# junliu111/CV-MonoSLAM

Measured on AMD Instinct MI355X. Metric: srukf_updates_per_sec, higher is better.
Workload: dtype f64; 1 GPU; BASELINE configs[2]: 200 inverse-depth landmarks (n=1204, Na=1209, L=2419), M=N matched, fp64, one batched refactor per frame, synthetic 640x480 figure-8 sequence; landmarks=200, state_dim=1204, sequences_per_gpu=1, update_mode=batched

## Files before the change

cv-monoslam_amd/csrc/srukf_rank.hip:

```cpp
#include <hip/hip_runtime.h>
#include "srukf_device.h"
#include "srukf_rank.h"
#include "srukf_motion.h"
#include "srukf_motion_reduce.h"
#include "srukf_launch.h"

__global__ __launch_bounds__(256) void k_rank_shadow(int n, int ld, int r, const double* __restrict__ S, const int* __restrict__ perm, double* __restrict__ A)
{
    const int a = blockIdx.x;
    double* out = A + (size_t)a * ld;
    if (a >= r) { for (int b = threadIdx.x; b < ld; b += 256) out[b] = 0.0; return; }
    const double* src = S + (size_t)perm[a] * ld;
    for (int b = threadIdx.x; b < ld; b += 256) out[b] = (b >= a && b < n) ? src[perm[b]] : 0.0;
}

__global__ __launch_bounds__(256) void k_row_energy(int n, int ld, const double* __restrict__ S, double* __restrict__ e)
{
    __shared__ double red[16];
    const int k = blockIdx.x;
    double v[1] = { 0.0 };
    for (int i = k + threadIdx.x; i < n; i += 256) { const double s = S[(size_t)k * ld + i]; v[0] += s * s; }
    block_sum<1>(v, red);
    if (threadIdx.x == 0) e[k] = v[0];
}

__global__ __launch_bounds__(256) void k_rank_diag(int n, int ld, const double* __restrict__ G, const int* __restrict__ perm, double* __restrict__ gdiag)
{
    const int a = blockIdx.x * 256 + threadIdx.x;
    if (a < n) { const int j = perm[a]; gdiag[a] = G[(size_t)j * ld + j]; }
}

template <int MODE>
__device__ __forceinline__ void rank_expand_body(int n, int ld, int r, double eps, const double* __restrict__ Sp, const double* __restrict__ D,
                                                 const int* __restrict__ perm, const int* __restrict__ iperm, const double* __restrict__ gdiag,
                                                 FrameScalars* __restrict__ fs, const double* __restrict__ X, int do_traj, double* __restrict__ S,
                                                 double* __restrict__ A, double* __restrict__ sigR, double gamma,
                                                 const KDims& d, const KWeights& w,
                                                 const srukf_params& p, double* __restrict__ Z, double* __restrict__ DZ, int f32, const int bid, const StepExport& ex, const double null_rel = 0.0,
                                                 unsigned int* __restrict__ fold_sync = nullptr, const int fold_words = 0)
{
    constexpr bool PROJ = MODE == 2;
    auto rnd = [&](double v) { return f32 ? (double)(float)v : v; };
    extern __shared__ double lrow[];
    __shared__ double prow[2][8];
    __shared__ double red[16 * 3];
    const int j = bid;
    const int Na = n + 5;
    const bool table = sigR && fs->ctl_next_valid && !fs->frozen;
    auto table_rows = [&](const int i, const int sg, const double (&srow)[4], const double (&mnoise)[3], const bool isnull) {
        const MotionCtl mc = { fs->ctl[0], fs->ctl[1], fs->ctl[2], fs->ctl[3], fs->ctl[4] };
        const double xr[4] = { X[n - 4], X[n - 3], X[n - 2], X[n - 1] };
        double rr[4], c2, s2;
        if (isnull) srukf_motion_centre(mc, xr, rr, c2, s2);
        else srukf_motion_point(mc, xr, srow, mnoise, sg ? -gamma : gamma, rr, c2, s2);
        double4* o = reinterpret_cast<double4*>(sigR + (size_t)(1 + sg * Na + i) * 8);
        o[0] = make_double4(rr[0], rr[1], rr[2], rr[3]); o[1] = make_double4(c2, s2, 0.0, 0.0);
        if constexpr (PROJ) { double* q = prow[sg]; q[0] = rr[0]; q[1] = rr[1]; q[2] = rr[2]; q[3] = rr[3]; q[4] = c2; q[5] = s2; }
    };
    const double f1 = PROJ ? p.cam_f / p.cam_dx : 0.0, f2 = PROJ ? p.cam_f / p.cam_dy : 0.0;
    auto project_pair = [&](const int i, const int k, const double (&dev)[6], const double e0, const double e1, const double* r0, const double* r1, const int dzrow) {
        double base[6];
#pragma unroll
        for (int e = 0; e < 6; e++) base[e] = X[6 * k + e];
        double zp[2], zm[2];
        srukf_project_sigma(p, f1, f2, base, dev, e0, e1, gamma, r0, zp[0], zp[1]);
        srukf_project_sigma(p, f1, f2, base, dev, e0, e1, -gamma, r1, zm[0], zm[1]);
        *reinterpret_cast<double2*>(Z + (size_t)(1 + i) * d.mp + 2 * k) = make_double2(zp[0], zp[1]);
        *reinterpret_cast<double2*>(Z + (size_t)(1 + Na + i) * d.mp + 2 * k) = make_double2(zm[0], zm[1]);
        if (dzrow >= 0) *reinterpret_cast<double2*>(DZ + (size_t)dzrow * d.mp + 2 * k) = make_double2(zp[0] - zm[0], zp[1] - zm[1]);
    };
    if constexpr (PROJ) {
        const int nchk = (n - r + SRUKF_RANK_COLS - 1) / SRUKF_RANK_COLS;
        if (j > n + nchk) {
            if (!table) return;
            const int q = j - n - nchk - 1;
            if (threadIdx.x < 2) {
                const double zero4[4] = { 0, 0, 0, 0 };
                double mnoise[3] = { 0, 0, 0 };
                if (q < 3) mnoise[q] = fs->ctl[5 + q];
                table_rows(n + q, threadIdx.x, zero4, mnoise, false);
            }
            __syncthreads();
            const double zero6[6] = { 0, 0, 0, 0, 0, 0 };
            const double e0 = (q == 3) ? p.sigma_measure : 0.0, e1 = (q == 4) ? p.sigma_measure : 0.0;
            for (int k = threadIdx.x; k < d.N; k += 256) project_pair(n + q, k, zero6, e0, e1, prow[0], prow[1], -1);
            return;
        }
    }
    if (j == n) {
        if (fold_sync) {
            const int base = (fold_words + FOLD_FLAG_STRIDE - 1) / FOLD_FLAG_STRIDE * FOLD_FLAG_STRIDE;
            for (int q = threadIdx.x; q < fold_words; q += 256) fold_sync[q] = 0u;
            if (threadIdx.x < 2 + SRUKF_STAT_GROUPS) fold_sync[base + FOLD_FLAG_STRIDE * threadIdx.x] = 0u;
        }
        if (table && threadIdx.x < (PROJ ? 1 : 11)) {
            const double zero4[4] = { 0, 0, 0, 0 };
            if (threadIdx.x == 0) {
                const MotionCtl mc = { fs->ctl[0], fs->ctl[1], fs->ctl[2], fs->ctl[3], fs->ctl[4] };
                const double xr[4] = { X[n - 4], X[n - 3], X[n - 2], X[n - 1] };
                double s0[4], c0s, s0s;
                srukf_motion_centre(mc, xr, s0, c0s, s0s);
                double4* o = reinterpret_cast<double4*>(sigR);
                o[0] = make_double4(s0[0], s0[1], s0[2], s0[3]); o[1] = make_double4(c0s, s0s, 0.0, 0.0);
                if constexpr (PROJ) { double* q = prow[0]; q[0] = s0[0]; q[1] = s0[1]; q[2] = s0[2]; q[3] = s0[3]; q[4] = c0s; q[5] = s0s; }
            } else {
                const int q = (threadIdx.x - 1) >> 1, sg = (threadIdx.x - 1) & 1;
                double mnoise[3] = { 0, 0, 0 };
                if (q < 3) mnoise[q] = fs->ctl[5 + q];
                table_rows(n + q, sg, zero4, mnoise, false);
            }
        }
        if constexpr (PROJ) {
            __syncthreads();
            if (table) {
                const double f1c = p.cam_f / p.cam_dx, f2c = p.cam_f / p.cam_dy;
                for (int k = threadIdx.x; k < d.N; k += 256) {
                    double base[6];
#pragma unroll
                    for (int e = 0; e < 6; e++) base[e] = X[6 * k + e];
                    double ox, oy;
                    srukf_project(p, f1c, f2c, base, prow[0][0], prow[0][1], prow[0][2], prow[0][4], prow[0][5], 0.0, 0.0, ox, oy);
                    *reinterpret_cast<double2*>(Z + 2 * k) = make_double2(ox, oy);
                }
            }
        }
        const int bx = iperm[n - 4], by = iperm[n - 3];
        double v[3] = { 0, 0, 0 };
        for (int a = threadIdx.x; a < r; a += 256) {
            const double p = (bx >= a) ? rnd(Sp[(size_t)a * ld + bx]) : 0.0, q = (by >= a) ? rnd(Sp[(size_t)a * ld + by]) : 0.0;
            v[0] += p * p; v[1] += p * q; v[2] += q * q;
        }
        block_sum<3>(v, red);
        if (ex.dst) {
            __shared__ double red4[16 * 10];
            int bc[4];
#pragma unroll
            for (int e = 0; e < 4; e++) bc[e] = iperm[n - 4 + e];
            double v4[10];
#pragma unroll
            for (int q = 0; q < 10; q++) v4[q] = 0.0;
            for (int a = threadIdx.x; a < r; a += 256) {
                double s4[4];
#pragma unroll
                for (int e = 0; e < 4; e++) s4[e] = (bc[e] >= a) ? rnd(Sp[(size_t)a * ld + bc[e]]) : 0.0;
                int q = 0;
#pragma unroll
                for (int e = 0; e < 4; e++)
#pragma unroll
                    for (int g = e; g < 4; g++) v4[q++] += s4[e] * s4[g];
            }
            block_sum<10>(v4, red4);
            if (threadIdx.x == 0) {
                int q = 0;
                for (int e = 0; e < 4; e++)
                    for (int g = e; g < 4; g++) { st_dev(ex.view + 4 * e + g, v4[q]); st_dev(ex.view + 4 * g + e, v4[q]); q++; }
                for (int e = 0; e < 4; e++) st_dev(ex.view + 16 + e, X[n - 4 + e]);
            }
        }
        if (threadIdx.x == 0 && do_traj) {
            double* traj = fs->traj_base;
            if (traj) {
                double* t = traj + (size_t)8 * fs->frame;
                for (int e = 0; e < 4; e++) t[e] = X[n - 4 + e];
                t[4] = v[0]; t[5] = v[1]; t[6] = v[1]; t[7] = v[2];
            }
            if (ex.dst) {
                __hip_atomic_store(&fs->frame, fs->frame + 1, __ATOMIC_RELAXED, __HIP_MEMORY_SCOPE_AGENT);
                __hip_atomic_store(&fs->const_rows_pending, 1, __ATOMIC_RELAXED, __HIP_MEMORY_SCOPE_AGENT);
            } else {
                fs->frame += 1;
                fs->const_rows_pending = 1;
            }
            if (!sigR) srukf_prepare_control(fs);
        }
        return;
    }
    if (j > n) {
        const int a = r + SRUKF_RANK_COLS * (j - n - 1) + (threadIdx.x & 15), kl = threadIdx.x >> 4;
        __shared__ double cs[16][17];
        cs[kl][threadIdx.x & 15] = (a < n) ? srukf_rank_colsq(Sp, ld, r, a, kl) : 0.0;
        __syncthreads();
        if (threadIdx.x < 16 && a < n) {
            double t = 0.0;
            for (int q = 0; q < 16; q++) t += cs[q][threadIdx.x];
            if (gdiag[a] - t > 1e-12 + null_rel * fabs(gdiag[a])) { atomicAdd(&fs->clamp_rows, 1); atomicMin(&fs->clamp_first, perm[a]); }
        }
        return;
    }
    const int a = j;
    const int jj = perm[a];
    double* out = S + (size_t)jj * ld;
    if (table && threadIdx.x < 2) {
        double srow[4] = { 0, 0, 0, 0 };
        const double zero3[3] = { 0, 0, 0 };
        if (a < r) {
#pragma unroll
            for (int e = 0; e < 4; e++) srow[e] = (r - 4 + e >= a) ? rnd(Sp[(size_t)a * ld + (r - 4 + e)]) : 0.0;
        }
        table_rows(jj, threadIdx.x, srow, zero3, a >= r);
    }
    if (a >= r) {
        if constexpr (PROJ) {
            if (table) {
                __syncthreads();
                if (threadIdx.x < 2) {
                    const int k = jj / 6, sg = threadIdx.x;
                    double dev[6], base[6];
#pragma unroll
                    for (int e = 0; e < 6; e++) { dev[e] = (6 * k + e == jj) ? rnd(sqrt(eps)) : 0.0; base[e] = X[6 * k + e]; }
                    double ox, oy;
                    srukf_project_sigma(p, f1, f2, base, dev, 0.0, 0.0, sg ? -gamma : gamma, prow[sg], ox, oy);
                    *reinterpret_cast<double2*>(Z + (size_t)(1 + sg * Na + jj) * d.mp + 2 * k) = make_double2(ox, oy);
                    const double pox = __shfl_xor(ox, 1), poy = __shfl_xor(oy, 1);
                    if (sg == 0) *reinterpret_cast<double2*>(DZ + (size_t)a * d.mp + 2 * k) = make_double2(ox - pox, oy - poy);
                }
            }
        }
        if (sigR && fs->const_rows_ok) return;
        for (int c = threadIdx.x; c < ld; c += 256) out[c] = (c == jj) ? rnd(sqrt(eps)) : 0.0;
        return;
    }
    const double* src = Sp + (size_t)a * ld;
    double* sh = A ? A + (size_t)a * ld : nullptr;
    double mx = 0.0;
    for (int b0 = (sigR ? (a & ~3) : 0) + threadIdx.x; b0 < ld; b0 += 4 * 256) {
        double sv[4]; int cc[4];
#pragma unroll
        for (int u = 0; u < 4; u++) {
            const int b = b0 + 256 * u;
            sv[u] = (b >= a && b < n) ? src[b] : 0.0;
            cc[u] = (b < n) ? perm[b] : b;
        }
#pragma unroll
        for (int u = 0; u < 4; u++) {
            const int b = b0 + 256 * u;
            if (b >= ld) break;
            const bool upper = b >= a && b < n && cc[u] >= jj;
            if (upper && cc[u] > jj) mx = fmax(mx, fabs(sv[u]));
            const double rv = rnd(sv[u]);
            if (sh) sh[b] = rv;
            if constexpr (PROJ) lrow[b] = rv;
            if (upper || !sigR) out[cc[u]] = upper ? rv : 0.0;
        }
    }
    mx = wave_max(mx);
    if ((threadIdx.x & 63) == 0) red[threadIdx.x >> 6] = mx;
    __syncthreads();
    if (threadIdx.x == 0) {
        mx = fmax(fmax(red[0], red[1]), fmax(red[2], red[3]));
        const double gamma = __longlong_as_double((long long)fs->gmax_bits);
        const double xi = __longlong_as_double((long long)fs->ximax_bits);
        const double nu = fmax(1.0, sqrt((double)n * n - 1.0));
        const double beta2 = fmax(fmax(gamma, xi / nu), 1e-15);
        const double dj = D[a];
        const double th = mx * sqrt(dj);
        if (th * th / beta2 > dj) { atomicAdd(&fs->clamp_rows, 1); atomicMin(&fs->clamp_first, jj); }
    }
    if constexpr (PROJ) {
        if (table) {
            for (int k = threadIdx.x; k < d.N; k += 256) {
                double dev[6];
#pragma unroll
                for (int e = 0; e < 6; e++) { const int col = 6 * k + e; dev[e] = (col >= jj) ? lrow[iperm[col]] : 0.0; }
                project_pair(jj, k, dev, 0.0, 0.0, prow[0], prow[1], a);
            }
        }
    }
}

template <int MODE>
__global__ __launch_bounds__(256) void k_rank_expand(int n, int ld, int r, double eps, const double* __restrict__ Sp, const double* __restrict__ D,
                                                     const int* __restrict__ perm, const int* __restrict__ iperm, const double* __restrict__ gdiag,
                                                     FrameScalars* __restrict__ fs, const double* __restrict__ X, int do_traj, double* __restrict__ S,
                                                     double* __restrict__ A, double* __restrict__ sigR, double gamma,
                                                     KDims d, KWeights w,
                                                     srukf_params p, double* __restrict__ Z, double* __restrict__ DZ, int f32, StepExport ex, double null_rel,
                                                     unsigned int* __restrict__ fold_sync, int fold_words)
{
    const int extra = (int)gridDim.x - n;
    const int bid = (int)blockIdx.x < extra ? n + (int)blockIdx.x : (int)blockIdx.x - extra;
    rank_expand_body<MODE>(n, ld, r, eps, Sp, D, perm, iperm, gdiag, fs, X, do_traj, S, A, sigR, gamma, d, w, p, Z, DZ, f32, bid, ex, null_rel, fold_sync, fold_words);
    if (!ex.dst) return;
    const int ncount = extra + r;
    if ((int)blockIdx.x >= ncount) return;
    __shared__ int last;
    asm volatile("s_waitcnt vmcnt(0)" ::: "memory");
    __syncthreads();
    if (threadIdx.x == 0) {
        const int g = (int)blockIdx.x & 63, gsize = (ncount - g + 63) >> 6, groups = ncount < 64 ? ncount : 64;
        int* c1 = ex.cnt + 64 * g;
        last = 0;
        if (__hip_atomic_fetch_add(c1, 1, __ATOMIC_RELAXED, __HIP_MEMORY_SCOPE_AGENT) == gsize - 1) {
            __hip_atomic_store(c1, 0, __ATOMIC_RELAXED, __HIP_MEMORY_SCOPE_AGENT);
            if (__hip_atomic_fetch_add(&fs->export_cnt, 1, __ATOMIC_RELAXED, __HIP_MEMORY_SCOPE_AGENT) == groups - 1) {
                __hip_atomic_store(&fs->export_cnt, 0, __ATOMIC_RELAXED, __HIP_MEMORY_SCOPE_AGENT);
                last = 1;
            }
        }
    }
    __syncthreads();
    if (!last) return;
    const unsigned long long* fw = (const unsigned long long*)fs;
    for (int i = threadIdx.x; i < ex.nfs; i += 256) ex.dst[i] = __hip_atomic_load(fw + i, __ATOMIC_RELAXED, __HIP_MEMORY_SCOPE_AGENT);
    if (threadIdx.x < 20) ((double*)(ex.dst + ex.nfs))[threadIdx.x] = ld_dev(ex.view + threadIdx.x);
    __threadfence_system();
    __syncthreads();
    if (threadIdx.x == 0) {
        if (ex.set && __hip_atomic_load(&fs->clamp_rows, __ATOMIC_RELAXED, __HIP_MEMORY_SCOPE_AGENT) == 0) {
            for (int e = 0; e < 6; e++) ex.odo[e] = ex.poses[e];
            srukf_step_scalars(fs, ex.odo, 1, ex.a, false);
        }
        if (ex.flag) __hip_atomic_store(ex.flag, ex.seq, __ATOMIC_RELEASE, __HIP_MEMORY_SCOPE_SYSTEM);
    }
}
__global__ __launch_bounds__(256) void k_rank_expand_b(int n, int ld, int r, double eps, const ExpandArgs* __restrict__ tab, int per, double gamma, KDims d, KWeights w, srukf_params p)
{
    const int f = (int)blockIdx.x / per, bid = (int)blockIdx.x - f * per;
    const ExpandArgs a = tab[f];
    rank_expand_body<2>(n, ld, r, eps, a.Sp, a.D, a.perm, a.iperm, a.gdiag, a.fs, a.X, 1, a.S, a.A, a.sigR, gamma, d, w, p, a.Z, a.DZ, 0, bid, StepExport{});
}

__global__ __launch_bounds__(256) void k_rank_round(int ld, double* __restrict__ A)
{
    double* row = A + (size_t)blockIdx.x * ld;
    for (int b = blockIdx.x + threadIdx.x; b < ld; b += 256) row[b] = (double)(float)row[b];
}

extern "C" {
void srukf_launch_rank_round(hipStream_t st, int ld, int r, double* A)
{
    hipLaunchKernelGGL(k_rank_round, dim3(r), dim3(256), 0, st, ld, A);
}
void srukf_launch_row_energy(hipStream_t st, int n, int ld, const double* S, double* e)
{
    hipLaunchKernelGGL(k_row_energy, dim3(n), dim3(256), 0, st, n, ld, S, e);
}
void srukf_launch_rank_diag(hipStream_t st, int n, int ld, const double* G, const int* perm, double* gdiag)
{
    hipLaunchKernelGGL(k_rank_diag, dim3((n + 255) / 256), dim3(256), 0, st, n, ld, G, perm, gdiag);
}
void srukf_launch_rank_expand(hipStream_t st, const RankExpandLaunch& a)
{
    const int n = a.d.n, ld = a.d.np, r = a.r, do_traj = a.do_traj ? 1 : 0;
    const bool fuse = a.fuse;
    const double eps = a.p.epsilon;
    const StepExport ex = (a.step_export && fuse) ? *a.step_export : StepExport{};
    const int nchk = (n - r + SRUKF_RANK_COLS - 1) / SRUKF_RANK_COLS;
    const dim3 grid(n + 1 + nchk + (fuse ? 5 : 0));
    if (fuse) hipLaunchKernelGGL(k_rank_expand<2>, grid, dim3(256), sizeof(double) * (size_t)ld, st, n, ld, r, eps, a.Sp, a.D, a.perm, a.iperm, a.gdiag, a.fs, a.X, do_traj, a.S, a.A, a.sigR, a.w.gamma, a.d, a.w, a.p, a.Z, a.DZ, a.f32round ? 1 : 0, ex, a.null_rel, a.fold_sync, a.fold_words);
    else hipLaunchKernelGGL(k_rank_expand<0>, grid, dim3(256), 0, st, n, ld, r, eps, a.Sp, a.D, a.perm, a.iperm, a.gdiag, a.fs, a.X, do_traj, a.S, a.A, a.sigR, a.w.gamma, a.d, a.w, a.p, a.Z, a.DZ, 0, StepExport{}, a.null_rel, a.fold_sync, a.fold_words);
}
void srukf_launch_rank_expand_b(hipStream_t st, int n, int ld, int r, double eps, const ExpandArgs* tab, int B, double gamma, KDims d, KWeights w, srukf_params p)
{
    const int nchk = (n - r + SRUKF_RANK_COLS - 1) / SRUKF_RANK_COLS;
    const int per = n + 1 + nchk + 5;
    hipLaunchKernelGGL(k_rank_expand_b, dim3(per * B), dim3(256), sizeof(double) * (size_t)ld, st, n, ld, r, eps, tab, per, gamma, d, w, p);
}
__global__ __launch_bounds__(256) void k_rank_canon(int n, int ld, int r, double sq, const int* __restrict__ perm, double* __restrict__ S)
{
    const int k = perm[r + blockIdx.x];
    if (k < 0 || k >= n) return;
    for (int c = threadIdx.x; c < ld; c += 256) S[(size_t)k * ld + c] = (c == k) ? sq : 0.0;
}
void srukf_launch_rank_canon(hipStream_t st, int n, int ld, int r, double sq, const int* perm, double* S)
{
    if (n - r > 0) hipLaunchKernelGGL(k_rank_canon, dim3(n - r), dim3(256), 0, st, n, ld, r, sq, perm, S);
}
void srukf_launch_rank_shadow(hipStream_t st, int n, int ld, int r, const double* S, const int* perm, double* A)
{
    hipLaunchKernelGGL(k_rank_shadow, dim3(ld), dim3(256), 0, st, n, ld, r, S, perm, A);
}
}
```

Measured before the change: 5604 frames/s.

## Split sigma-point projection out of per-row expand blocks into packed tail blocks

Sigma-point projection was previously done inside each of the n row blocks, one block looping over all landmarks per row, with a shared-memory copy of the row. It is now done by dedicated blocks that flatten (row, landmark) pairs across 256-512 threads, plus separate blocks for null rows and for canonical-row fills. The motion sigma points for each row are precomputed into LDS. This shrinks the dynamic shared memory and spreads the projection work evenly across the grid. In exchange it adds more blocks, rereads Sp from global memory, and makes the completion-counter indexing more complex.

New measurement: 5590 frames/s. No clear change (-0.3%).

```diff
diff --git a/cv-monoslam_amd/csrc/srukf_rank.hip b/cv-monoslam_amd/csrc/srukf_rank.hip
--- a/cv-monoslam_amd/csrc/srukf_rank.hip
+++ b/cv-monoslam_amd/csrc/srukf_rank.hip
@@ -28,6 +28,37 @@
 {
     const int a = blockIdx.x * 256 + threadIdx.x;
     if (a < n) { const int j = perm[a]; gdiag[a] = G[(size_t)j * ld + j]; }
+}
+
+#define SRUKF_TAIL_DROP_BLOCKS 32
+struct TailGrid {
+    int extra, pb, nb, rows, db;
+    __host__ __device__ int total() const { return extra + pb + nb + rows + db; }
+    __host__ __device__ int counted() const { return extra + rows; }
+    __host__ __device__ static int chunks(int N) { return N > 256 ? 2 : 1; }
+    __host__ __device__ static int block_rows(int N) { return 256 * chunks(N) / N + 2; }
+    __host__ __device__ static size_t lds_bytes(int N) { return sizeof(double) * 12 * (size_t)block_rows(N); }
+};
+__host__ __device__ inline TailGrid tail_grid(int n, int r, int N)
+{
+    const int nchk = (n - r + SRUKF_RANK_COLS - 1) / SRUKF_RANK_COLS;
+    TailGrid g;
+    g.extra = 1 + nchk + 5;
+    g.pb = (int)(((long long)r * N + 256 * TailGrid::chunks(N) - 1) / (256 * TailGrid::chunks(N)));
+    g.nb = (2 * (n - r) + 255) / 256;
+    g.rows = r;
+    g.db = n - r < SRUKF_TAIL_DROP_BLOCKS ? n - r : SRUKF_TAIL_DROP_BLOCKS;
+    return g;
+}
+__device__ __forceinline__ int tail_bid(const TailGrid& g, int n, int b)
+{
+    const int packed = g.extra + g.pb + g.nb;
+    return b < packed ? n + b : b < packed + g.rows ? b - packed : n + b - g.rows;
+}
+__device__ __forceinline__ int tail_counted(const TailGrid& g, int b)
+{
+    const int packed = g.extra + g.pb + g.nb;
+    return b < g.extra ? b : (b >= packed && b < packed + g.rows) ? b - (g.pb + g.nb) : -1;
 }
 
 template <int MODE>
@@ -41,7 +72,7 @@
 {
     constexpr bool PROJ = MODE == 2;
     auto rnd = [&](double v) { return f32 ? (double)(float)v : v; };
-    extern __shared__ double lrow[];
+    extern __shared__ double mpts[];
     __shared__ double prow[2][8];
     __shared__ double red[16 * 3];
     const int j = bid;
@@ -58,10 +89,7 @@
         if constexpr (PROJ) { double* q = prow[sg]; q[0] = rr[0]; q[1] = rr[1]; q[2] = rr[2]; q[3] = rr[3]; q[4] = c2; q[5] = s2; }
     };
     const double f1 = PROJ ? p.cam_f / p.cam_dx : 0.0, f2 = PROJ ? p.cam_f / p.cam_dy : 0.0;
-    auto project_pair = [&](const int i, const int k, const double (&dev)[6], const double e0, const double e1, const double* r0, const double* r1, const int dzrow) {
-        double base[6];
-#pragma unroll
-        for (int e = 0; e < 6; e++) base[e] = X[6 * k + e];
+    auto project_pair = [&](const int i, const int k, const double (&base)[6], const double (&dev)[6], const double e0, const double e1, const double* r0, const double* r1, const int dzrow) {
         double zp[2], zm[2];
         srukf_project_sigma(p, f1, f2, base, dev, e0, e1, gamma, r0, zp[0], zp[1]);
         srukf_project_sigma(p, f1, f2, base, dev, e0, e1, -gamma, r1, zm[0], zm[1]);
@@ -70,6 +98,97 @@
         if (dzrow >= 0) *reinterpret_cast<double2*>(DZ + (size_t)dzrow * d.mp + 2 * k) = make_double2(zp[0] - zm[0], zp[1] - zm[1]);
     };
     if constexpr (PROJ) {
+        const TailGrid tg = tail_grid(n, r, d.N);
+        if (j >= n + tg.extra) {
+            int q = j - n - tg.extra;
+            if (q < tg.pb) {
+                const int N = d.N, M = TailGrid::chunks(N), j0 = 256 * M * q;
+                const int a0 = j0 / N, nr = min(r - 1, (j0 + 256 * M - 1) / N) - a0 + 1;
+                int jb = j0 + (int)threadIdx.x;
+                bool live = jb < r * N;
+                int a = live ? jb / N : r - 1, k = live ? jb - a * N : 0;
+                int jj = perm[a];
+                int bc[6];
+                double base[6], dev[6], srow[4];
+#pragma unroll
+                for (int e = 0; e < 6; e++) { bc[e] = iperm[6 * k + e]; base[e] = X[6 * k + e]; }
+                const bool mlane = (int)threadIdx.x < 2 * nr;
+                const int ar0 = a0 + ((int)threadIdx.x >> 1);
+#pragma unroll
+                for (int e = 0; e < 4; e++) srow[e] = (mlane && r - 4 + e >= ar0) ? rnd(Sp[(size_t)ar0 * ld + (r - 4 + e)]) : 0.0;
+                if (!table) return;
+#pragma unroll
+                for (int e = 0; e < 6; e++) dev[e] = (6 * k + e >= jj && bc[e] >= a && bc[e] < n) ? rnd(Sp[(size_t)a * ld + bc[e]]) : 0.0;
+                const MotionCtl mc = { fs->ctl[0], fs->ctl[1], fs->ctl[2], fs->ctl[3], fs->ctl[4] };
+                const double xr[4] = { X[n - 4], X[n - 3], X[n - 2], X[n - 1] };
+                for (int t = threadIdx.x; t < 2 * nr; t += 256) {
+                    const int ar = a0 + (t >> 1), sg = t & 1;
+                    double rr[4], c2, s2;
+                    const double zero3[3] = { 0, 0, 0 };
+                    if (t >= 256) {
+#pragma unroll
+                        for (int e = 0; e < 4; e++) srow[e] = (r - 4 + e >= ar) ? rnd(Sp[(size_t)ar * ld + (r - 4 + e)]) : 0.0;
+                    }
+                    srukf_motion_point(mc, xr, srow, zero3, sg ? -gamma : gamma, rr, c2, s2);
+                    double* o = mpts + 6 * t;
+                    o[0] = rr[0]; o[1] = rr[1]; o[2] = rr[2]; o[3] = rr[3]; o[4] = c2; o[5] = s2;
+                }
+                __syncthreads();
+                if (live) project_pair(jj, k, base, dev, 0.0, 0.0, mpts + 12 * (a - a0), mpts + 12 * (a - a0) + 6, a);
+                for (int m = 1; m < M; m++) {
+                    jb += 256;
+                    if (jb >= r * N) break;
+                    a = jb / N; k = jb - a * N; jj = perm[a];
+#pragma unroll
+                    for (int e = 0; e < 6; e++) { bc[e] = iperm[6 * k + e]; base[e] = X[6 * k + e]; }
+#pragma unroll
+                    for (int e = 0; e < 6; e++) dev[e] = (6 * k + e >= jj && bc[e] >= a && bc[e] < n) ? rnd(Sp[(size_t)a * ld + bc[e]]) : 0.0;
+                    project_pair(jj, k, base, dev, 0.0, 0.0, mpts + 12 * (a - a0), mpts + 12 * (a - a0) + 6, a);
+                }
+                return;
+            }
+            q -= tg.pb;
+            if (q < tg.nb) {
+                const int jn = 256 * q + (int)threadIdx.x, a = r + (jn >> 1), sg = jn & 1;
+                const bool live = a < n;
+                const int jj = perm[live ? a : n - 1], k = jj / 6;
+                double base[6];
+#pragma unroll
+                for (int e = 0; e < 6; e++) base[e] = X[6 * k + e];
+                if (!table) return;
+                if (threadIdx.x == 0) {
+                    const MotionCtl mc = { fs->ctl[0], fs->ctl[1], fs->ctl[2], fs->ctl[3], fs->ctl[4] };
+                    const double xr[4] = { X[n - 4], X[n - 3], X[n - 2], X[n - 1] };
+                    double rr[4], c2, s2;
+                    srukf_motion_centre(mc, xr, rr, c2, s2);
+                    double* o = prow[0];
+                    o[0] = rr[0]; o[1] = rr[1]; o[2] = rr[2]; o[3] = rr[3]; o[4] = c2; o[5] = s2;
+                }
+                __syncthreads();
+                double ox = 0.0, oy = 0.0;
+                if (live) {
+                    const double* c0 = prow[0];
+                    double4* o = reinterpret_cast<double4*>(sigR + (size_t)(1 + sg * Na + jj) * 8);
+                    o[0] = make_double4(c0[0], c0[1], c0[2], c0[3]); o[1] = make_double4(c0[4], c0[5], 0.0, 0.0);
+                    double dev[6];
+#pragma unroll
+                    for (int e = 0; e < 6; e++) dev[e] = (6 * k + e == jj) ? rnd(sqrt(eps)) : 0.0;
+                    srukf_project_sigma(p, f1, f2, base, dev, 0.0, 0.0, sg ? -gamma : gamma, c0, ox, oy);
+                    *reinterpret_cast<double2*>(Z + (size_t)(1 + sg * Na + jj) * d.mp + 2 * k) = make_double2(ox, oy);
+                }
+                const double pox = __shfl_xor(ox, 1), poy = __shfl_xor(oy, 1);
+                if (live && sg == 0) *reinterpret_cast<double2*>(DZ + (size_t)a * d.mp + 2 * k) = make_double2(ox - pox, oy - poy);
+                return;
+            }
+            q -= tg.nb;
+            if (sigR && fs->const_rows_ok) return;
+            for (int a = r + q; a < n; a += tg.db) {
+                const int jj = perm[a];
+                double* out = S + (size_t)jj * ld;
+                for (int c = threadIdx.x; c < ld; c += 256) out[c] = (c == jj) ? rnd(sqrt(eps)) : 0.0;
+            }
+            return;
+        }
         const int nchk = (n - r + SRUKF_RANK_COLS - 1) / SRUKF_RANK_COLS;
         if (j > n + nchk) {
             if (!table) return;
@@ -83,7 +202,12 @@
             __syncthreads();
             const double zero6[6] = { 0, 0, 0, 0, 0, 0 };
             const double e0 = (q == 3) ? p.sigma_measure : 0.0, e1 = (q == 4) ? p.sigma_measure : 0.0;
-            for (int k = threadIdx.x; k < d.N; k += 256) project_pair(n + q, k, zero6, e0, e1, prow[0], prow[1], -1);
+            for (int k = threadIdx.x; k < d.N; k += 256) {
+                double base[6];
+#pragma unroll
+                for (int e = 0; e < 6; e++) base[e] = X[6 * k + e];
+                project_pair(n + q, k, base, zero6, e0, e1, prow[0], prow[1], -1);
+            }
             return;
         }
     }
@@ -200,22 +324,6 @@
         table_rows(jj, threadIdx.x, srow, zero3, a >= r);
     }
     if (a >= r) {
-        if constexpr (PROJ) {
-            if (table) {
-                __syncthreads();
-                if (threadIdx.x < 2) {
-                    const int k = jj / 6, sg = threadIdx.x;
-                    double dev[6], base[6];
-#pragma unroll
-                    for (int e = 0; e < 6; e++) { dev[e] = (6 * k + e == jj) ? rnd(sqrt(eps)) : 0.0; base[e] = X[6 * k + e]; }
-                    double ox, oy;
-                    srukf_project_sigma(p, f1, f2, base, dev, 0.0, 0.0, sg ? -gamma : gamma, prow[sg], ox, oy);
-                    *reinterpret_cast<double2*>(Z + (size_t)(1 + sg * Na + jj) * d.mp + 2 * k) = make_double2(ox, oy);
-                    const double pox = __shfl_xor(ox, 1), poy = __shfl_xor(oy, 1);
-                    if (sg == 0) *reinterpret_cast<double2*>(DZ + (size_t)a * d.mp + 2 * k) = make_double2(ox - pox, oy - poy);
-                }
-            }
-        }
         if (sigR && fs->const_rows_ok) return;
         for (int c = threadIdx.x; c < ld; c += 256) out[c] = (c == jj) ? rnd(sqrt(eps)) : 0.0;
         return;
@@ -239,7 +347,6 @@
             if (upper && cc[u] > jj) mx = fmax(mx, fabs(sv[u]));
             const double rv = rnd(sv[u]);
             if (sh) sh[b] = rv;
-            if constexpr (PROJ) lrow[b] = rv;
             if (upper || !sigR) out[cc[u]] = upper ? rv : 0.0;
         }
     }
@@ -256,16 +363,6 @@
         const double th = mx * sqrt(dj);
         if (th * th / beta2 > dj) { atomicAdd(&fs->clamp_rows, 1); atomicMin(&fs->clamp_first, jj); }
     }
-    if constexpr (PROJ) {
-        if (table) {
-            for (int k = threadIdx.x; k < d.N; k += 256) {
-                double dev[6];
-#pragma unroll
-                for (int e = 0; e < 6; e++) { const int col = 6 * k + e; dev[e] = (col >= jj) ? lrow[iperm[col]] : 0.0; }
-                project_pair(jj, k, dev, 0.0, 0.0, prow[0], prow[1], a);
-            }
-        }
-    }
 }
 
 template <int MODE>
@@ -277,17 +374,23 @@
                                                      srukf_params p, double* __restrict__ Z, double* __restrict__ DZ, int f32, StepExport ex, double null_rel,
                                                      unsigned int* __restrict__ fold_sync, int fold_words)
 {
-    const int extra = (int)gridDim.x - n;
-    const int bid = (int)blockIdx.x < extra ? n + (int)blockIdx.x : (int)blockIdx.x - extra;
+    int bid, cidx, ncount;
+    if constexpr (MODE == 2) {
+        const TailGrid tg = tail_grid(n, r, d.N);
+        bid = tail_bid(tg, n, (int)blockIdx.x); cidx = tail_counted(tg, (int)blockIdx.x); ncount = tg.counted();
+    } else {
+        const int extra = (int)gridDim.x - n;
+        bid = (int)blockIdx.x < extra ? n + (int)blockIdx.x : (int)blockIdx.x - extra;
+        ncount = extra + r; cidx = (int)blockIdx.x < ncount ? (int)blockIdx.x : -1;
+    }
     rank_expand_body<MODE>(n, ld, r, eps, Sp, D, perm, iperm, gdiag, fs, X, do_traj, S, A, sigR, gamma, d, w, p, Z, DZ, f32, bid, ex, null_rel, fold_sync, fold_words);
     if (!ex.dst) return;
-    const int ncount = extra + r;
-    if ((int)blockIdx.x >= ncount) return;
+    if (cidx < 0) return;
     __shared__ int last;
     asm volatile("s_waitcnt vmcnt(0)" ::: "memory");
     __syncthreads();
     if (threadIdx.x == 0) {
-        const int g = (int)blockIdx.x & 63, gsize = (ncount - g + 63) >> 6, groups = ncount < 64 ? ncount : 64;
+        const int g = cidx & 63, gsize = (ncount - g + 63) >> 6, groups = ncount < 64 ? ncount : 64;
         int* c1 = ex.cnt + 64 * g;
         last = 0;
         if (__hip_atomic_fetch_add(c1, 1, __ATOMIC_RELAXED, __HIP_MEMORY_SCOPE_AGENT) == gsize - 1) {
@@ -315,7 +418,7 @@
 }
 __global__ __launch_bounds__(256) void k_rank_expand_b(int n, int ld, int r, double eps, const ExpandArgs* __restrict__ tab, int per, double gamma, KDims d, KWeights w, srukf_params p)
 {
-    const int f = (int)blockIdx.x / per, bid = (int)blockIdx.x - f * per;
+    const int f = (int)blockIdx.x / per, bid = tail_bid(tail_grid(n, r, d.N), n, (int)blockIdx.x - f * per);
     const ExpandArgs a = tab[f];
     rank_expand_body<2>(n, ld, r, eps, a.Sp, a.D, a.perm, a.iperm, a.gdiag, a.fs, a.X, 1, a.S, a.A, a.sigR, gamma, d, w, p, a.Z, a.DZ, 0, bid, StepExport{});
 }
@@ -346,15 +449,14 @@
     const double eps = a.p.epsilon;
     const StepExport ex = (a.step_export && fuse) ? *a.step_export : StepExport{};
     const int nchk = (n - r + SRUKF_RANK_COLS - 1) / SRUKF_RANK_COLS;
-    const dim3 grid(n + 1 + nchk + (fuse ? 5 : 0));
-    if (fuse) hipLaunchKernelGGL(k_rank_expand<2>, grid, dim3(256), sizeof(double) * (size_t)ld, st, n, ld, r, eps, a.Sp, a.D, a.perm, a.iperm, a.gdiag, a.fs, a.X, do_traj, a.S, a.A, a.sigR, a.w.gamma, a.d, a.w, a.p, a.Z, a.DZ, a.f32round ? 1 : 0, ex, a.null_rel, a.fold_sync, a.fold_words);
+    const dim3 grid(fuse ? tail_grid(n, r, a.d.N).total() : n + 1 + nchk);
+    if (fuse) hipLaunchKernelGGL(k_rank_expand<2>, grid, dim3(256), TailGrid::lds_bytes(a.d.N), st, n, ld, r, eps, a.Sp, a.D, a.perm, a.iperm, a.gdiag, a.fs, a.X, do_traj, a.S, a.A, a.sigR, a.w.gamma, a.d, a.w, a.p, a.Z, a.DZ, a.f32round ? 1 : 0, ex, a.null_rel, a.fold_sync, a.fold_words);
     else hipLaunchKernelGGL(k_rank_expand<0>, grid, dim3(256), 0, st, n, ld, r, eps, a.Sp, a.D, a.perm, a.iperm, a.gdiag, a.fs, a.X, do_traj, a.S, a.A, a.sigR, a.w.gamma, a.d, a.w, a.p, a.Z, a.DZ, 0, StepExport{}, a.null_rel, a.fold_sync, a.fold_words);
 }
 void srukf_launch_rank_expand_b(hipStream_t st, int n, int ld, int r, double eps, const ExpandArgs* tab, int B, double gamma, KDims d, KWeights w, srukf_params p)
 {
-    const int nchk = (n - r + SRUKF_RANK_COLS - 1) / SRUKF_RANK_COLS;
-    const int per = n + 1 + nchk + 5;
-    hipLaunchKernelGGL(k_rank_expand_b, dim3(per * B), dim3(256), sizeof(double) * (size_t)ld, st, n, ld, r, eps, tab, per, gamma, d, w, p);
+    const int per = tail_grid(n, r, d.N).total();
+    hipLaunchKernelGGL(k_rank_expand_b, dim3(per * B), dim3(256), TailGrid::lds_bytes(d.N), st, n, ld, r, eps, tab, per, gamma, d, w, p);
 }
 __global__ __launch_bounds__(256) void k_rank_canon(int n, int ld, int r, double sq, const int* __restrict__ perm, double* __restrict__ S)
 {
```
